# NVIDIA-Genomics-Research/DL4VC

Hardware: AMD Instinct MI355X
Metric: candidate-variants/sec (DAN fwd, 64 reads x 201 bp) (higher is better)
Workload: dtype f32

## Files before the change

dl4vc_amd/config.py:

```python
from __future__ import annotations

from dataclasses import dataclass, field, asdict
from typing import Sequence, Tuple

SINGLE_READ_LENGTH = 201
NUM_SINGLE_READS = 100
MAX_READS = 100
MIN_RESIDUAL_LAYER = 2
MAX_LAYERS = 16
L0_MAX_LAYERS = 12

PRECISION_F32 = 0
PRECISION_BF16X3 = 1
PRECISION_BF16 = 2


class UnsupportedModelOption(ValueError):
    """A Basic2DNet option outside the hot path's scope was requested."""


@dataclass(frozen=True)
class DanConfig:
    reads: int = NUM_SINGLE_READS
    length: int = SINGLE_READ_LENGTH
    layers: int = 7
    c_init: int = 128
    c_final: int = 128
    dil_mid: int = 2
    dil_final: int = 2
    pool_layers: Tuple[int, ...] = (2,)
    residual_start: int = 5
    use_bn: bool = True
    use_q: bool = True
    use_strand: bool = True
    use_mask: bool = True
    bottleneck: int = 32
    fc_sizes: Tuple[int, ...] = (1024, 256)
    embed_dim: int = 20
    precision: int = PRECISION_F32
    conv_algo: int = 0
    skip_empty_rows: bool = False
    bf16_form: int = 0

# ... 24 lines not shown
    @property
    def highway_width(self) -> int:
        return self.layers * self.bottleneck * self.reads

    @property
    def feature_width(self) -> int:
        return self.pooled_width + self.highway_width

    def macs_per_position(self) -> int:
        total = 0
        for l in range(1, self.layers + 1):
            cin, cout, _ = self.layer_dims(l)
            total += 3 * cin * cout
            if self.is_residual(l):
                total += cout * cout
            total += cout * self.bottleneck + self.bottleneck * self.bottleneck
        return total

    def flops_per_site(self) -> float:
        fc = 0
        sizes = (self.feature_width,) + tuple(self.fc_sizes)
        for a, b in zip(sizes[:-1], sizes[1:]):
            fc += a * b
        fc += sizes[-1] * 27
        return 2.0 * (self.reads * self.length * self.macs_per_position() + fc)

    def winograd_applies(self) -> bool:
        dil_ok = (self.layers < 3 or self.dil_mid == 2) and (self.layers < 2 or self.dil_final == 2)
        return self.precision == PRECISION_F32 and dil_ok and self.conv_algo != 1 and self.layers > 1

    def executed_macs_per_position(self) -> float:
        total = float(self.macs_per_position())
        if self.winograd_applies():
            for l in range(2, self.layers + 1):
                cin, cout, _ = self.layer_dims(l)
                total -= cin * cout
        first_segment = min(self.pool_layers) if self.pool_layers else self.layers
        if self.precision == PRECISION_F32 and first_segment <= L0_MAX_LAYERS:
            cin, cout, _ = self.layer_dims(1)
            total -= 3 * cin * cout
        return total

    def input_bytes_per_site(self) -> int:
        return 3 * self.reads * self.length + 3 * self.length

    def to_dict(self):
        return asdict(self)

    def validate(self):
        if not (1 <= self.layers <= MAX_LAYERS):
            raise UnsupportedModelOption("layers must be in 1..%d" % MAX_LAYERS)
        if self.reads < 1 or self.length < 8:
            raise UnsupportedModelOption("reads >= 1 and length >= 8 required")
        if self.residual_start > 0 and self.residual_start < MIN_RESIDUAL_LAYER:
            raise UnsupportedModelOption("Do not allow residuals starting at conv layer %d" % self.residual_start)
        for p in self.pool_layers:
            if not (1 <= p < self.layers):
                raise UnsupportedModelOption("pool layer %d must lie in 1..layers-1" % p)
        if self.layers == 1 and self.c_init != self.c_final:
            raise UnsupportedModelOption("a single conv layer needs init_conv_channels == final_conv_channels")
        if self.bottleneck < 0 or len(self.fc_sizes) != 2:
            raise UnsupportedModelOption("bottleneck >= 0 and exactly two FC layers required")
        if self.conv_algo not in (0, 1, 2):
            raise UnsupportedModelOption("conv_algo must be 0 (auto), 1 (direct) or 2 (winograd)")
        if self.bf16_form not in (0, 1) or (self.bf16_form and self.precision != PRECISION_BF16):
            raise UnsupportedModelOption("bf16_form is 0 or 1 and selects a form of the precision-2 (bf16) kernel")
        if self.embed_dim != 20:
            raise UnsupportedModelOption("embed_dim is fixed at 20 in the reference's scripts")

# ... 39 lines not shown
```

dl4vc_amd/csrc/dan_capi.cpp:

```cpp
#include "../../include/dl4vc_dan.h"
#include "dan_kernels.h"

#include <algorithm>
#include <cmath>
#include <cstdarg>
#include <cstdio>
#include <cstring>
#include <map>
#include <string>
#include <thread>
#include <vector>

using namespace dan;

namespace {

struct Tensor {
    std::vector<float> data;
    std::vector<int64_t> shape;
    int64_t numel() const { int64_t n = 1; for (auto s : shape) n *= s; return n; }
};

std::string g_create_error;

// ... 388 lines not shown
                        v += (double)s.Wf(o, e, t) * emb.data[(size_t)ta * EMBED + e] + (double)s.Wf(o, EMBED + e, t) * emb.data[(size_t)tb * EMBED + e];
                    tab[L0_TJ_OFF + ((size_t)t * L0_NTJ + ta * 10 + tb) * CPAD + o] = (float)v;
                }
            for (int k = 0; k < 5; ++k) tab[L0_WSC_OFF + ((size_t)k * 3 + t) * CPAD + o] = s.Wf(o, 2 * EMBED + k, t);
        }
    std::vector<double> pet((size_t)3 * L * CPAD);
    for (int t = 0; t < 3; ++t)
        for (int wcol = 0; wcol < L; ++wcol)
            for (int o = 0; o < CPAD; ++o) {
                double v = 0.0;
                for (int e = 0; e < EMBED; ++e) v += ((double)s.Wf(o, e, t) + (double)s.Wf(o, EMBED + e, t)) * pe.data[(size_t)wcol * EMBED + e];
                pet[((size_t)t * L + wcol) * CPAD + o] = v;
            }
    for (int var = 0; var < 3; ++var)
        for (int wcol = 0; wcol < L; ++wcol)
            for (int o = 0; o < CPAD; ++o) {
                double v = pet[((size_t)1 * L + wcol) * CPAD + o];
                if (var != 1 && wcol - 1 >= 0) v += pet[((size_t)0 * L + wcol - 1) * CPAD + o];
                if (var != 2 && wcol + 1 < L) v += pet[((size_t)2 * L + wcol + 1) * CPAD + o];
                tab[L0_PE_OFF + ((size_t)var * L + wcol) * CPAD + o] = (float)v;
            }
    return tab;
}

void pack_layer_fp32(const LayerSrc& s, float* blk) {
    auto Wf = [&](int o, int cc, int t) { return s.Wf(o, cc, t); };
    pack_frag(blk + W_OFF, 3, s.l == 0 ? KG0 : KGC, KGC, Wf);
    if (s.l > 0) {
        auto Wu = [&](int o, int cc, int k) -> float {
            const double g0 = s.Wf(o, cc, 0), g1 = s.Wf(o, cc, 1), g2 = s.Wf(o, cc, 2);
            return k == 0 ? (float)g0 : k == 1 ? (float)((g0 + g1 + g2) * 0.5) : k == 2 ? (float)((g0 - g1 + g2) * 0.5) : (float)g2;
        };
        pack_frag(blk + WW_OFF, 4, KGC, KGC, Wu);
    }
    if (s.wr) pack_frag(blk + WRES_OFF, 1, KGC, KGC, [&](int o, int cc, int) { return s.Wr(o, cc); });
    if (s.wb) pack_frag(blk + WBOT_OFF, 1, KGC, 2, [&](int o, int cc, int) { return s.Wb(o, cc); });
}

void pack_layer_bf16p(const LayerSrc& s, const float* cst, char* blkp, char* blkr) {
    auto Wf = [&](int o, int cc, int t) { return s.Wf(o, cc, t); };
    auto Wr = [&](int o, int cc, int) { return s.Wr(o, cc); };
    auto Wb = [&](int o, int cc, int) { return s.Wb(o, cc); };
    pack_fragp((uint16_t*)(blkp + WP_CONV_OFF), 3, s.l == 0 ? P_KS0 : P_KSC, 4, Wf);
    pack_frag16<1>((uint16_t*)(blkr + WP_CONV_OFF), 3, s.l == 0 ? 2 : 4, 8, Wf);
    if (s.wr) {
        pack_fragp((uint16_t*)(blkp + WP_RES_OFF), 1, P_KSC, 4, Wr);
        pack_frag16<1>((uint16_t*)(blkr + WP_RES_OFF), 1, 4, 8, Wr);
    }
    if (s.wb) {
        pack_fragp((uint16_t*)(blkp + WP_BOT_OFF), 1, P_KSC, 1, Wb);
        pack_frag16<1>((uint16_t*)(blkr + WP_BOT_OFF), 1, 4, 2, Wb);
    }
    memcpy(blkp + WP_CST_OFF, cst, CST_FLOATS * sizeof(float));
    memcpy(blkr + WP_CST_OFF, cst, CST_FLOATS * sizeof(float));
}

void pack_layer_bf16x(const LayerSrc& s, const float* cst, char* blkx) {
    pack_frag16<2>((uint16_t*)(blkx + WX_CONV_OFF), 3, s.l == 0 ? X_KS0 : X_KS, 8, [&](int o, int cc, int t) { return s.Wf(o, cc, t); });
    if (s.wr) pack_frag16<2>((uint16_t*)(blkx + WX_RES_OFF), 1, X_KS, 8, [&](int o, int cc, int) { return s.Wr(o, cc); });
    if (s.wb) pack_frag16<2>((uint16_t*)(blkx + WX_BOT_OFF), 1, X_KS, 2, [&](int o, int cc, int) { return s.Wb(o, cc); });
    float* cx = (float*)(blkx + WX_CST_OFF);
    memcpy(cx, cst, CST_FLOATS * sizeof(float));
    for (int ch = 0; ch < CPAD; ++ch) {
        const double b = cx[CST_BIAS + ch];
        cx[CST_SHIFT + ch] = (float)((double)cx[CST_SHIFT + ch] + b * (double)cx[CST_SCALE + ch]);
        cx[CST_BIAS + ch] = (float)-b;
// ... 593 lines not shown
}

int dan_set_tap(dan_t* h, int32_t layer) {
    if (!h) return DAN_ERR_INVALID_ARG;
    if (layer < -1 || layer > h->cfg.layers) return fail(h, DAN_ERR_INVALID_ARG, "tap layer %d out of range", layer);
    if (layer >= 0 && !h->d_tap) {
        if (!h->finalized) return fail(h, DAN_ERR_STATE, "dan_set_tap before dan_finalize");
        HIPCHK(h, hipSetDevice(h->cfg.device_id));
        int rc = dev_alloc(h, &h->d_tap, (size_t)h->chunk * h->cfg.reads * h->cfg.length * CPAD);
        if (rc) return rc;
    }
    h->tap_layer = layer;
    return DAN_OK;
}

int dan_set_pool_form(dan_t* h, int32_t form) {
    if (!h) return DAN_ERR_INVALID_ARG;
    if (form < 0 || form > 2) return fail(h, DAN_ERR_INVALID_ARG, "pool form %d: 0 = automatic, 1 = separate kernels, 2 = in-segment", form);
    if (form == 2 && h->fold_why_not) return fail(h, DAN_ERR_INVALID_ARG, "pool form 2 refused: %s", h->fold_why_not);
    h->pool_form = form;
    h->last_pool_form = (form == 1 || h->fold_why_not) ? 1 : 2;
    return DAN_OK;
}

int64_t dan_query(const dan_t* h, const char* what) {
    if (!h || !what) return DAN_ERR_INVALID_ARG;
    const std::string w(what);
    if (w == "feature_width") return h->F;
    if (w == "feature_stride") return h->F_stride;
    if (w == "chunk_sites") return h->chunk;
    if (w == "chunk_sites_auto") return h->chunk_auto ? 1 : 0;
    if (w == "max_batch") return h->max_batch;
    if (w == "cpad") return CPAD;
    if (w == "tap_sites") return h->last_chunk_sites;
    if (w == "segments") return h->n_segments;
    if (w == "bf16_pingpong") return h->fam == &FAMILIES[2] ? 1 : 0;
    if (w == "bf16x3_split_kernel") return h->fam == &FAMILIES[1] ? 1 : 0;
    if (w == "hidden0_stride") return h->n0_stride;
    if (w == "pool_form") return h->last_pool_form;
    return fail(h, DAN_ERR_INVALID_ARG, "dan_query: unknown key '%s'", what);
}

int64_t dan_read_buffer(dan_t* h, const char* name, float* dst, int64_t capacity) {
    if (!h || !name || !dst || capacity < 0) return DAN_ERR_INVALID_ARG;
    if (!h->finalized) return fail(h, DAN_ERR_STATE, "dan_read_buffer before dan_finalize");
    const dan_config& c = h->cfg;
    const std::string w(name);
    const float* src = nullptr;
    int64_t n = 0;
    if (w == "tap") { if (!h->d_tap) return fail(h, DAN_ERR_STATE, "no tap was requested"); src = h->d_tap; n = (int64_t)h->last_chunk_sites * c.reads * c.length * CPAD; }
    else if (w == "feature") { src = h->d_feat; n = h->last_batch * h->F_stride; }
    else if (w == "hidden0") { src = h->d_hid0; n = h->last_batch * h->n0_stride; }
    else if (w == "hidden1") { src = h->d_hid1; n = h->last_batch * c.fc_sizes[1]; }
    else if (w == "pool") { src = h->d_pool; n = (int64_t)h->last_chunk_sites * c.length * CPAD; }
    else if (w == "h") {
        if (!h->d_h) return fail(h, DAN_ERR_STATE, "the network has no highway bottleneck");
        const int64_t per_layer = (int64_t)h->last_chunk_sites * c.reads * c.length * HPAD;
        const int64_t stride = (int64_t)h->chunk * c.reads * c.length * HPAD;
        if (per_layer == 0) return fail(h, DAN_ERR_STATE, "dan_read_buffer('h') before the first forward");
        if (capacity < per_layer)
            return fail(h, DAN_ERR_INVALID_ARG, "dan_read_buffer('h'): capacity %lld is less than one layer (%lld floats)", (long long)capacity,
                        (long long)per_layer);
        n = std::min<int64_t>(per_layer * c.layers, capacity) / per_layer * per_layer;
        HIPCHK(h, hipSetDevice(c.device_id));
        HIPCHK(h, hipDeviceSynchronize());
        const bool h_bf16 = h->fam->elem_bytes == 2;
        std::vector<uint16_t> tmp(h_bf16 ? (size_t)per_layer : 0);
        for (int64_t l = 0; l * per_layer < n; ++l) {
            if (h_bf16) {
                HIPCHK(h, hipMemcpy(tmp.data(), (const uint16_t*)h->d_h + l * stride, (size_t)per_layer * 2, hipMemcpyDeviceToHost));
                for (int64_t i = 0; i < per_layer; ++i) dst[l * per_layer + i] = bf16_float(tmp[(size_t)i]);
            } else {
                HIPCHK(h, hipMemcpy(dst + l * per_layer, h->d_h + l * stride, (size_t)per_layer * sizeof(float), hipMemcpyDeviceToHost));
            }
        }
        return n;
    }
    else return fail(h, DAN_ERR_INVALID_ARG, "dan_read_buffer: unknown buffer '%s'", name);
    n = std::min(n, capacity);
    HIPCHK(h, hipSetDevice(c.device_id));
    HIPCHK(h, hipDeviceSynchronize());
    HIPCHK(h, hipMemcpy(dst, src, (size_t)n * sizeof(float), hipMemcpyDeviceToHost));
    return n;
}

int dan_profile_enable(dan_t* h, int32_t on) {
// ... 23 lines not shown
```

dl4vc_amd/csrc/dan_device.h:

```cpp
#pragma once
#include "dan_kernels.h"

namespace dan {

typedef float v4f __attribute__((ext_vector_type(4)));

__device__ __forceinline__ v4f mfma16(float a, float b, v4f c) {
    return __builtin_amdgcn_mfma_f32_16x16x4f32(a, b, c, 0, 0, 0);
}

__device__ __forceinline__ v4f splat(float x) { return (v4f){x, x, x, x}; }

typedef const __attribute__((address_space(1))) v4f* gv4f_ptr;

__device__ __forceinline__ float relu1(float v) { return __builtin_amdgcn_fmed3f(v, 0.f, __builtin_inff()); }

__device__ __forceinline__ void gemm_tile(v4f (&acc)[NT], const v4f (&a)[NT], v4f& b, const float* next) {
#pragma unroll
    for (int s = 0; s < 4; ++s)
#pragma unroll
        for (int n = 0; n < NT; ++n) acc[n] = mfma16(a[n][s], b[s], acc[n]);
    b = *(const v4f*)next;
}

__device__ __forceinline__ void conv_gemm(v4f (&acc)[MTW][NT], const float* xs, gv4f_ptr wl, const v4f (&a_first)[NT],
                                          int kg, int ntaps, int dil, int lane, int m_base, int cnt) {
    const int pos = lane & 15, kk = lane >> 4;
    const int total = ntaps * kg;
    const int t0 = (ntaps == 3) ? -dil : 0;
    const float* xrow = xs + (HALO + m_base * 16 + pos) * LDS_S + kk * 4;
    const bool full = cnt == MTW;
    v4f a_nxt[NT], b[MTW];
#pragma unroll
    for (int n = 0; n < NT; ++n) a_nxt[n] = a_first[n];
    {
        const float* xb = xrow + t0 * LDS_S;
#pragma unroll
        for (int m = 0; m < MTW - 1; ++m) b[m] = *(const v4f*)(xb + m * 16 * LDS_S);
        b[MTW - 1] = full ? *(const v4f*)(xb + (MTW - 1) * 16 * LDS_S) : splat(0.f);
    }
    int t = 0, g = 0;
    for (int it = 0; it < total; ++it) {
        v4f a[NT];
#pragma unroll
        for (int n = 0; n < NT; ++n) a[n] = a_nxt[n];
        const int nx = (it + 1 < total) ? it + 1 : it;
#pragma unroll
        for (int n = 0; n < NT; ++n) a_nxt[n] = wl[(size_t)nx * (KGC * 64) + n * 64];
        int tn = t, gn = g + 1;
        if (gn == kg) { gn = 0; ++tn; }
        if (it + 1 == total) { tn = t; gn = g; }
        const float* xn = xrow + (t0 + tn * dil) * LDS_S + gn * 16;
#pragma unroll
        for (int m = 0; m < MTW - 1; ++m) gemm_tile(acc[m], a, b[m], xn + m * 16 * LDS_S);
        __builtin_amdgcn_sched_group_barrier(0x020, NT, 0);
#pragma unroll
        for (int m = 0; m < MTW - 1; ++m) {
            __builtin_amdgcn_sched_group_barrier(0x008, 4 * NT, 0);
            __builtin_amdgcn_sched_group_barrier(0x100, 1, 0);
        }
        if (full) gemm_tile(acc[MTW - 1], a, b[MTW - 1], xn + (MTW - 1) * 16 * LDS_S);
        t = tn; g = gn;
    }
}

template <int NW, bool RANGE = false, int TILES = MT>
__device__ __forceinline__ void bottleneck(const float* xs, const v4f (&wf)[KGC], const float* bbot, float* hrow, int L,
                                           int wave, int lane, int p_lo = 0) {
    constexpr int PSTEP = NW / 2;
    constexpr int NBT = (TILES + PSTEP - 1) / PSTEP;
    lane = (int)__builtin_amdgcn_mbcnt_hi(~0u, __builtin_amdgcn_mbcnt_lo(~0u, 0u));
    asm volatile("" : "+v"(lane));
    const int pos = lane & 15, kk = lane >> 4;
    const int n = wave & 1, p0 = wave >> 1;
    const float* xrow = xs + (HALO + pos) * LDS_S + kk * 4;
    int roff[NBT];
#pragma unroll
    for (int i = 0; i < NBT; ++i) roff[i] = min(p0 + PSTEP * i, TILES - 1) * 16 * LDS_S;
    v4f acc[NBT], b[NBT];
    {
        const v4f bias = *(const v4f*)(bbot + n * 16 + kk * 4);
#pragma unroll
        for (int i = 0; i < NBT; ++i) acc[i] = bias;
    }
#pragma unroll
    for (int i = 0; i < NBT; ++i) b[i] = *(const v4f*)(xrow + roff[i]);
#pragma unroll
    for (int g = 0; g < KGC; ++g) {
        const int gn = (g + 1 < KGC) ? g + 1 : g;
#pragma unroll
        for (int i = 0; i < NBT; ++i) {
#pragma unroll
            for (int s = 0; s < 4; ++s) acc[i] = mfma16(wf[g][s], b[i][s], acc[i]);
            b[i] = *(const v4f*)(xrow + roff[i] + gn * 16);
// ... 14 lines not shown
            *(v4f*)((char*)hrow + (unsigned)(p * HPAD + n * 16 + kk * 4) * 4u) = v;
        }
    }
}

__device__ __forceinline__ void copy_out(const float* xs, float* dst, int lo, int hi, int tid) {
    for (int i = lo * (CPAD / 4) + tid; i < hi * (CPAD / 4); i += SEG_THREADS) {
        const int p = i >> 5, c4 = i & 31;
        ((v4f*)dst)[i] = *(const v4f*)(xs + (HALO + p) * LDS_S + c4 * 4);
    }
}

constexpr int MW = 7;
constexpr int WHB = 102;
constexpr int MW_SHORT = 6;
constexpr int WHB_SHORT = 94;
constexpr int MPOS_SHORT = WHB_SHORT + 16 * MW_SHORT;
constexpr int wino_half_base(int tw) { return tw == MW ? WHB : WHB_SHORT; }
constexpr int wino_cover(int tw) { return tw == MW ? MPOS : MPOS_SHORT; }
template <int TW = MW>
__device__ __forceinline__ int wino_base(int lane) {
    const int n = lane & 15;
    const int c = n & 1, hf = (n >> 2) & 1, q = ((n >> 1) & 1) + 2 * (((n >> 3) ^ (n >> 2)) & 1);
    return hf * wino_half_base(TW) + 4 * q * TW + c;
}

typedef float v2f __attribute__((ext_vector_type(2)));
__device__ __forceinline__ v4f pk_sub(v4f a, v4f b, v2f m1) {
    const v2f lo = __builtin_elementwise_fma((v2f){b[0], b[1]}, m1, (v2f){a[0], a[1]});
    const v2f hi = __builtin_elementwise_fma((v2f){b[2], b[3]}, m1, (v2f){a[2], a[3]});
    return (v4f){lo[0], lo[1], hi[0], hi[1]};
}
__device__ __forceinline__ v4f pk_add(v4f a, v4f b) { return a + b; }
template <int TW, bool REM = false>
__device__ __forceinline__ void conv_gemm_wino(v4f (&acc)[TW][4], const float* xrow, gv4f_ptr wl, const v4f (&a_first)[4],
                                               [[maybe_unused]] v4f& racc, [[maybe_unused]] const float* xr, [[maybe_unused]] gv4f_ptr wd) {
    static_assert(!REM || TW == 6, "the remainder tile's taps follow tiles 1, 3 and 5 of a six-tile walk");
    v4f a_nxt[4];
#pragma unroll
    for (int k = 0; k < 4; ++k) a_nxt[k] = a_first[k];
    v4f xa = *(const v4f*)(xrow), xb = *(const v4f*)(xrow + 2 * LDS_S), xc = *(const v4f*)(xrow + 4 * LDS_S),
        xd = *(const v4f*)(xrow + 6 * LDS_S);
    float neg1 = -1.f;
    asm volatile("" : "+v"(neg1));
    const v2f m1 = {neg1, neg1};
    for (int g = 0; g < KGC; ++g) {
        v4f a[4];
#pragma unroll
        for (int k = 0; k < 4; ++k) a[k] = a_nxt[k];
        const int gn = (g + 1 < KGC) ? g + 1 : g;
#pragma unroll
        for (int k = 0; k < 4; ++k) a_nxt[k] = wl[(size_t)(k * KGC + gn) * (KGC * 64)];
        [[maybe_unused]] v4f ra[3], rb;
        if constexpr (REM) {
#pragma unroll
            for (int t = 0; t < 3; ++t) ra[t] = wd[(size_t)(t * KGC + g) * (KGC * 64)];
        }
        const float* xg = xrow + g * 16;
        const float* xn = xrow + gn * 16;
#pragma unroll
        for (int m = 0; m < TW; ++m) {
            v4f v[4];
            v[0] = pk_sub(xa, xc, m1); v[1] = pk_add(xb, xc); v[2] = pk_sub(xc, xb, m1); v[3] = pk_sub(xb, xd, m1);
            if (m + 1 < TW) {
                xa = xc; xb = xd;
                xc = *(const v4f*)(xg + (4 * m + 8) * LDS_S);
                xd = *(const v4f*)(xg + (4 * m + 10) * LDS_S);
            } else {
                xa = *(const v4f*)(xn); xb = *(const v4f*)(xn + 2 * LDS_S);
                xc = *(const v4f*)(xn + 4 * LDS_S); xd = *(const v4f*)(xn + 6 * LDS_S);
            }
            if constexpr (REM) {
                if ((m & 1) == 0) rb = *(const v4f*)(xr + (m >> 1) * 2 * LDS_S + g * 16);
            }
            __builtin_amdgcn_s_setprio(3);
#pragma unroll
            for (int s = 0; s < 4; ++s)
#pragma unroll
                for (int k = 0; k < 4; ++k) acc[m][k] = mfma16(a[k][s], v[k][s], acc[m][k]);
            if constexpr (REM) {
                if (m & 1) {
#pragma unroll
                    for (int s = 0; s < 4; ++s) racc = mfma16(ra[m >> 1][s], rb[s], racc);
                }
            }
            __builtin_amdgcn_s_setprio(0);
        }
    }
}
template <int TW>
__device__ __forceinline__ void conv_gemm_wino(v4f (&acc)[TW][4], const float* xrow, gv4f_ptr wl, const v4f (&a_first)[4]) {
    v4f none = splat(0.f);
    conv_gemm_wino<TW, false>(acc, xrow, wl, a_first, none, nullptr, nullptr);
}

constexpr int WINO_ROWS_READ = HALO + WHB + 4 * (4 * MW - 1) + 1 + 4 + 1;

}
```

dl4vc_amd/csrc/dan_kernels.h:

```cpp
#pragma once
#include <hip/hip_runtime.h>
#include <stdint.h>

namespace dan {

constexpr int CPAD = 128;
constexpr int NWAVE = 8;
constexpr int SEG_THREADS = NWAVE * 64;
constexpr int NT = 2;
constexpr int MTW = 7;
constexpr int MT = 13;
constexpr int MPOS = MT * 16;
constexpr int HALO = 4;
constexpr int LDS_S = 136;
constexpr int LDS_ROWS = MPOS + 2 * HALO;
constexpr int HPAD = 32;
constexpr int CIN0 = 48;
constexpr int KG0 = CIN0 / 16;
constexpr int KGC = CPAD / 16;
constexpr int EMBED = 20;
constexpr int VOCAB = 10;
constexpr int NHEAD = 27;

constexpr int W_OFF = 0;
constexpr int WRES_OFF = W_OFF + 3 * KGC * KGC * 256;
constexpr int WBOT_OFF = WRES_OFF + KGC * KGC * 256;
constexpr int CST_OFF = WBOT_OFF + KGC * 2 * 256;
constexpr int CST_BIAS = 0, CST_SCALE = CPAD, CST_SHIFT = 2 * CPAD, CST_BRES = 3 * CPAD, CST_BBOT = 4 * CPAD;
constexpr int CST_FLOATS = 4 * CPAD + HPAD;
constexpr int WW_OFF = CST_OFF + CST_FLOATS + 32;
constexpr int LAYER_STRIDE = WW_OFF + 4 * KGC * KGC * 256;
constexpr int MAX_LAYERS = 16;

struct SegmentArgs {
    const float* wl;
    int l_begin, l_end;
    int n_layers;
    int dil_mid, dil_final;
    unsigned res_mask;
    int has_hw;
    int R, L;
    const uint8_t *reads, *qual, *strand, *ref, *ref_mask, *var_mask;
    const float* emb;
    const float* pe;
    float* y;
    const float* pool;
    float* h;
    long long h_layer_stride;
    float* tap;
    int tap_layer;
    int wino;
    int n_rows;
    int xcd_rows;
    const int* work;
    const int* work_count;
    const float* l0_tab;
    int units, Lw;
    int u_off[2], u_len[2], own_lo[2], own_hi[2];
    float* y_out;
    int fold;
    int n_sites, xcd_sites;
    float* fold_scratch;
    float* fold_pool;
    float* fold_feat;
// ... 142 lines not shown
```

dl4vc_amd/csrc/dan_kernels.hip:

```cpp
#include "dan_device.h"
#include "dan_reduce.h"

namespace dan {

#ifdef DAN_STAMPS
__device__ unsigned long long* g_stamps;
constexpr int NSTAMP = 64;
#define STAMP(k)                                                                                      \
    do {                                                                                              \
        __builtin_amdgcn_sched_barrier(0);                                                            \
        unsigned long long t_ = __builtin_amdgcn_s_memtime();                                         \
        __builtin_amdgcn_s_waitcnt(0xC07F);                                                           \
        if (lane == 0 && (k) < NSTAMP) g_stamps[((size_t)stamp_row * NWAVE + wave) * NSTAMP + (k)] = t_; \
        __builtin_amdgcn_sched_barrier(0);                                                            \
    } while (0)
#else
#define STAMP(k) do {} while (0)
#endif

static_assert((HALO + WHB + 4 * (4 * MW - 1) + 1 + 4 + 1) * LDS_S <= LDS_ROWS * LDS_S + MAX_LAYERS * CST_FLOATS, "wino reads stay inside LDS");
static_assert(WHB + 4 * (4 * MW - 1) + 3 >= MPOS - 1 && 4 * (4 * MW - 1) + 3 >= WHB - 1, "wino tiling covers the read");
static_assert(HALO + MPOS_SHORT + 15 + 2 < LDS_ROWS && MPOS_SHORT + 16 <= MPOS, "the remainder tile's taps stay inside the image");
static_assert(WHB_SHORT + 4 * (4 * MW_SHORT - 1) + 3 >= MPOS_SHORT - 1 && 4 * (4 * MW_SHORT - 1) + 3 >= WHB_SHORT - 1 && WHB_SHORT % 4 == 2,
              "short wino tiling covers its unit");
// ... 11 lines not shown
    for (int g = 0; g < KGC; ++g) {
        const v4f a = a_nxt;
        const int gn = (g + 1 < KGC) ? g + 1 : g;
        a_nxt = wl[(size_t)gn * (KGC * 64)];
#pragma unroll
        for (int m = 0; m < TW; ++m) {
            __builtin_amdgcn_s_setprio(3);
#pragma unroll
            for (int s = 0; s < 4; ++s)
#pragma unroll
                for (int o = 0; o < 2; ++o) acc[m][o] = mfma16(a[s], b[m][o][s], acc[m][o]);
            if constexpr (REM) {
                if (m + 1 == TW) {
#pragma unroll
                    for (int s = 0; s < 4; ++s) racc = mfma16(a[s], rb[s], racc);
                }
            }
            __builtin_amdgcn_s_setprio(0);
#pragma unroll
            for (int o = 0; o < 2; ++o) b[m][o] = *(const v4f*)(xrow + (4 * m + 2 * o) * LDS_S + gn * 16);
            if constexpr (REM) {
                if (m + 1 == TW) rb = *(const v4f*)(xr + gn * 16);
            }
        }
    }
}

template <bool WINO, bool PERSIST, bool SPLIT, int TW = MW, bool FOLD = false, bool REM = false>
__global__ __launch_bounds__(SEG_THREADS, NWAVE / 4) void segment_kernel(SegmentArgs a_by_value) {
    static_assert(!FOLD || (PERSIST && !SPLIT), "the site-owning form is a persistent one-unit form");
    static_assert(TW == MW ? !(SPLIT && WINO) : (WINO && TW == MW_SHORT), "six tiles per lane: Winograd forms only, and the split one always");
    static_assert(!REM || (WINO && !SPLIT && TW == MW_SHORT), "the remainder tile [190, 206): beside six Winograd tiles of a one-unit read");
    constexpr int TILES = (SPLIT && WINO) ? (MPOS_SHORT + 15) / 16 : MT;
    __shared__ __attribute__((aligned(16))) float lds[LDS_ROWS * LDS_S + MAX_LAYERS * CST_FLOATS];
    float* const xs = lds;
    float* const cst = lds + LDS_ROWS * LDS_S;
    typedef const __attribute__((address_space(4))) SegmentArgs* kernarg_ptr;
    constexpr int UNITS = SPLIT ? 2 : 1;
    const int n_work = FOLD ? a_by_value.n_sites : (a_by_value.work_count ? *a_by_value.work_count : a_by_value.n_rows) * UNITS;
    const int per = FOLD ? a_by_value.xcd_sites : a_by_value.work_count ? (n_work + 7) >> 3 : a_by_value.xcd_rows * UNITS;
    const int xcd = blockIdx.x & 7;
    int j = blockIdx.x >> 3;
    int wk = xcd * per + j;
    if (j >= per || wk >= n_work) return;
    [[maybe_unused]] int fold_r = 0;
next_row:
    {
    kernarg_ptr ap = (kernarg_ptr)__builtin_amdgcn_kernarg_segment_ptr();
    if (PERSIST) asm volatile("" : "+s"(ap));
    auto args = [&]() -> decltype(auto) { if constexpr (PERSIST) return (*ap); else return (a_by_value); };
    const auto& a = args();
    [[maybe_unused]] const int unit = wk & 1;
    const int L = SPLIT ? (unit ? a.u_len[1] : a.u_len[0]) : a.L;
    const int Lw = SPLIT ? a.Lw : L;
    const int u_off = SPLIT ? (unit ? a.u_off[1] : a.u_off[0]) : 0;
    [[maybe_unused]] const int own_lo = SPLIT ? (unit ? a.own_lo[1] : a.own_lo[0]) : 0;
    [[maybe_unused]] const int own_hi = SPLIT ? (unit ? a.own_hi[1] : a.own_hi[0]) : L;
    [[maybe_unused]] const int stamp_row = wk;
    int tid = threadIdx.x;
    if (PERSIST) asm volatile("" : "+v"(tid));
    const int lane = tid & 63;
    const int wave = __builtin_amdgcn_readfirstlane(tid >> 6);
    const int wrow = SPLIT ? wk >> 1 : wk;
    const int row_index = FOLD ? wk * a.R + fold_r : __builtin_amdgcn_readfirstlane(a.work_count ? a.work[wrow] : wrow);
    const int site = FOLD ? wk : (int)((unsigned)row_index / (unsigned)a.R);
    const int r = FOLD ? fold_r : row_index - site * a.R;
    const size_t read_idx = (size_t)site * a.R + r;
    float* yrow = a.y + (read_idx * (size_t)Lw + u_off) * CPAD;
    float* yout = SPLIT ? a.y_out + (read_idx * (size_t)Lw + u_off) * CPAD : yrow;
    const int pos = lane & 15, kk = lane >> 4;
    const int cq = wave & 3, ph = wave >> 2;
    const int m_base = ph * MTW, cnt = ph ? MT - MTW : MTW;
    int chb[NT];
#pragma unroll
    for (int n = 0; n < NT; ++n) chb[n] = (cq * NT + n) * 16 + kk * 4;

    STAMP(0);
    [[maybe_unused]] const int wP0 = wino_base<TW>(lane);
    [[maybe_unused]] const int wlim = ((lane >> 2) & 1) ? wino_cover(TW) : wino_half_base(TW);
    [[maybe_unused]] const int chw = wave * 16 + kk * 4;
    auto dil_of = [&](int l) { return (l == 0) ? 1 : (l + 1 < a.n_layers ? a.dil_mid : a.dil_final); };
    auto wino_layer = [&](int l) { return WINO && l > 0; };
    constexpr bool CARRY = !(WINO && PERSIST);
    v4f pc0 = splat(0.f), pc1 = pc0, pc2 = pc0, pc3 = pc0, pn0 = pc0, pn1 = pc0, pn2 = pc0, pn3 = pc0;
    auto first_frags = [&](int l, v4f& f0, v4f& f1, v4f& f2, v4f& f3) {
        const float* blk = a.wl + (size_t)l * LAYER_STRIDE;
        if (wino_layer(l)) {
            gv4f_ptr w0 = (gv4f_ptr)(blk + WW_OFF) + wave * 64 + lane;
            constexpr size_t KS = (size_t)KGC * (KGC * 64);
            f0 = w0[0]; f1 = w0[KS]; f2 = w0[2 * KS]; f3 = w0[3 * KS];
        } else {
            gv4f_ptr w0 = (gv4f_ptr)(blk + W_OFF) + (cq * NT) * 64 + lane;
            f0 = w0[0]; f1 = w0[64];
        }
    };
    const bool l0_lookup = a.l_begin == 0 && a.l0_tab != nullptr && !(a.tap && a.tap_layer == 0) && (a.l_end - a.l_begin) <= L0_MAX_LAYERS;
    float* const tokf = cst + (a.l_end - a.l_begin) * CST_FLOATS;
    if ((!WINO || a.l_begin == 0) && !l0_lookup) first_frags(a.l_begin, pc0, pc1, pc2, pc3);
    auto stage_constants = [&]() {
        for (int i = tid; i < (a.l_end - a.l_begin) * CST_FLOATS; i += SEG_THREADS) {
            const int l = i / CST_FLOATS, j = i - l * CST_FLOATS;
            cst[i] = a.wl[(size_t)(a.l_begin + l) * LAYER_STRIDE + CST_OFF + j];
        }
    };

    if (a.l_begin == 0) {
        if (l0_lookup) {
            for (int i = tid; i < (LDS_ROWS - L) * (LDS_S / 4); i += SEG_THREADS) {
                const int rr = i / (LDS_S / 4), c4 = i - rr * (LDS_S / 4);
                const int row = rr < HALO ? rr : rr + L;
                *(v4f*)(xs + row * LDS_S + c4 * 4) = splat(0.f);
            }
        } else {
            for (int i = tid; i < LDS_ROWS * LDS_S / 4; i += SEG_THREADS) ((v4f*)xs)[i] = splat(0.f);
        }
        stage_constants();
// ... 100 lines not shown
        STAMP(sb + 7);
        if (CARRY) { pc0 = pn0; pc1 = pn1; pc2 = pn2; pc3 = pn3; }
    };

    auto direct_layer = [&](int l) {
        const float* wblk = a.wl + (size_t)l * LAYER_STRIDE;
        const float* lc = cst + (l - a.l_begin) * CST_FLOATS;
        const bool residual = (a.res_mask >> l) & 1u;
        const int kg = (l == 0) ? KG0 : KGC;
        const int dil = dil_of(l);
        gv4f_ptr w_conv = (gv4f_ptr)(wblk + W_OFF) + (cq * NT) * 64 + lane;
        gv4f_ptr w_res = (gv4f_ptr)(wblk + WRES_OFF) + (cq * NT) * 64 + lane;
        gv4f_ptr w_bot = (gv4f_ptr)(wblk + WBOT_OFF) + lane;
        [[maybe_unused]] const int sb = 2 + (l - a.l_begin) * 8;
        if (!WINO && l + 1 < a.l_end) first_frags(l + 1, pn0, pn1, pn2, pn3);
        const bool from_global = (l == a.l_begin) && (a.l_begin != 0) && (a.pool != nullptr);
        v4f pre_res[NT];
#pragma unroll
        for (int n = 0; n < NT; ++n) pre_res[n] = residual ? w_res[n * 64] : splat(0.f);
        static_assert(NT == 2, "two direct-form fragments are carried");
        const v4f pre_dir[NT] = {pc0, pc1};

        v4f acc[MTW][NT];
        {
            v4f bias[NT];
#pragma unroll
            for (int n = 0; n < NT; ++n) bias[n] = *(const v4f*)(lc + CST_BIAS + chb[n]);
#pragma unroll
            for (int m = 0; m < MTW; ++m)
#pragma unroll
                for (int n = 0; n < NT; ++n) acc[m][n] = bias[n];
        }
        STAMP(sb + 0);
        conv_gemm(acc, xs, w_conv, pre_dir, kg, 3, dil, lane, m_base, cnt);
        STAMP(sb + 1);
        const bool bot_here = a.has_hw && !(WINO && l + 1 < a.l_end);
        if (bot_here && !residual) {
#pragma unroll
            for (int g = 0; g < KGC; ++g) wbot[g] = w_bot[(g * 2 + (wave & 1)) * 64];
        }
        {
            v4f sc[NT], sh[NT];
#pragma unroll
            for (int n = 0; n < NT; ++n) { sc[n] = *(const v4f*)(lc + CST_SCALE + chb[n]); sh[n] = *(const v4f*)(lc + CST_SHIFT + chb[n]); }
#pragma unroll
            for (int m = 0; m < MTW; ++m) {
                const bool live = ((m_base + m) * 16 + pos) < L;
#pragma unroll
                for (int n = 0; n < NT; ++n) {
                    v4f v = acc[m][n];
#pragma unroll
                    for (int j = 0; j < 4; ++j) v[j] = live ? relu1(v[j]) * sc[n][j] + sh[n][j] : 0.f;
                    acc[m][n] = v;
                }
            }
        }
        STAMP(sb + 2);
        __syncthreads();
        STAMP(sb + 3);
        if (residual) {
            v4f bres[NT];
#pragma unroll
            for (int n = 0; n < NT; ++n) bres[n] = *(const v4f*)(lc + CST_BRES + chb[n]);
            if (!from_global) {
#pragma unroll
                for (int m = 0; m < MTW; ++m) {
                    if (m < cnt) {
// ... 37 lines not shown
                    for (int n = 0; n < NT; ++n) *(v4f*)(xs + (HALO + p) * LDS_S + chb[n]) = (p < L) ? acc[m][n] : splat(0.f);
                }
            }
        } else {
#pragma unroll
            for (int m = 0; m < MTW; ++m) {
                if (m < cnt) {
#pragma unroll
                    for (int n = 0; n < NT; ++n)
                        *(v4f*)(xs + (HALO + (m_base + m) * 16 + pos) * LDS_S + chb[n]) = acc[m][n];
                }
            }
        }
        layer_tail(l, lc, true);
    };

    [[maybe_unused]] auto wino_layer_body = [&](int l) {
        if constexpr (WINO) {
        const float* wblk = a.wl + (size_t)l * LAYER_STRIDE;
        const float* lc = cst + (l - a.l_begin) * CST_FLOATS;
        const bool residual = (a.res_mask >> l) & 1u;
        gv4f_ptr w_bot = (gv4f_ptr)(wblk + WBOT_OFF) + lane;
        [[maybe_unused]] const int sb = 2 + (l - a.l_begin) * 8;
        const bool from_global = (l == a.l_begin) && (a.l_begin != 0) && (a.pool != nullptr);
        gv4f_ptr w_w = (gv4f_ptr)(wblk + WW_OFF) + wave * 64 + lane;
        gv4f_ptr w_r1 = (gv4f_ptr)(wblk + WRES_OFF) + wave * 64 + lane;
        float* xw = xs + (HALO + wP0) * LDS_S;
        v4f out[TW][2], pre_r1;
        [[maybe_unused]] v4f rout = splat(0.f);
        [[maybe_unused]] int rp = MPOS_SHORT + pos;
        int wp = wP0;
        float* xq;
        {
            v4f acc[TW][4];
            const v4f bias = *(const v4f*)(lc + CST_BIAS + chw);
#pragma unroll
            for (int m = 0; m < TW; ++m) { acc[m][0] = splat(0.f); acc[m][1] = bias; acc[m][2] = splat(0.f); acc[m][3] = splat(0.f); }
            if constexpr (REM) rout = bias;
            STAMP(sb + 0);
            auto gemm = [&](const v4f (&pre_w)[4]) {
                if constexpr (REM)
                    conv_gemm_wino<TW, true>(acc, xw - 2 * LDS_S + kk * 4, w_w, pre_w, rout, xs + (HALO + rp - 2) * LDS_S + kk * 4, (gv4f_ptr)(wblk + W_OFF) + wave * 64 + lane);
                else
                    conv_gemm_wino(acc, xw - 2 * LDS_S + kk * 4, w_w, pre_w);
            };
            if constexpr (CARRY) {
                const v4f pre_w[4] = {pc0, pc1, pc2, pc3};
                gemm(pre_w);
            } else {
                gv4f_ptr w0 = w_w;
                const v4f pre_w[4] = {w0[0], w0[(size_t)KGC * (KGC * 64)], w0[(size_t)2 * KGC * (KGC * 64)], w0[(size_t)3 * KGC * (KGC * 64)]};
                gemm(pre_w);
            }
            STAMP(sb + 1);
            asm volatile("" : "+v"(wp));
            if constexpr (REM) asm volatile("" : "+v"(rp));
            xq = xs + (HALO + wp) * LDS_S;
            const v4f sc = *(const v4f*)(lc + CST_SCALE + chw), sh = *(const v4f*)(lc + CST_SHIFT + chw);
            const v2f sc_lo = {sc[0], sc[1]}, sc_hi = {sc[2], sc[3]}, sh_lo = {sh[0], sh[1]}, sh_hi = {sh[2], sh[3]};
            auto half = [](v4f v, int h) { return (v2f){v[2 * h], v[2 * h + 1]}; };
            v2f neg1 = {-1.f, -1.f};
            asm volatile("" : "+v"(neg1));
            auto act = [](v2f y, v2f s, v2f t) {
                const v2f r = {relu1(y[0]), relu1(y[1])};
                return __builtin_elementwise_fma(r, s, t);
            };
#pragma unroll
            for (int m = 0; m < TW; ++m) {
                const v2f y0l = half(acc[m][0], 0) + half(acc[m][1], 0) + half(acc[m][2], 0), y0h = half(acc[m][0], 1) + half(acc[m][1], 1) + half(acc[m][2], 1);
                const v2f y1l = __builtin_elementwise_fma(half(acc[m][3], 0), neg1, __builtin_elementwise_fma(half(acc[m][2], 0), neg1, half(acc[m][1], 0)));
                const v2f y1h = __builtin_elementwise_fma(half(acc[m][3], 1), neg1, __builtin_elementwise_fma(half(acc[m][2], 1), neg1, half(acc[m][1], 1)));
                const v2f o0l = act(y0l, sc_lo, sh_lo), o0h = act(y0h, sc_hi, sh_hi), o1l = act(y1l, sc_lo, sh_lo), o1h = act(y1h, sc_hi, sh_hi);
                out[m][0] = (v4f){o0l[0], o0l[1], o0h[0], o0h[1]};
                out[m][1] = (v4f){o1l[0], o1l[1], o1h[0], o1h[1]};
            }
            if constexpr (REM) {
                const v2f rl = act(half(rout, 0), sc_lo, sh_lo), rh = act(half(rout, 1), sc_hi, sh_hi);
                rout = (v4f){rl[0], rl[1], rh[0], rh[1]};
            }
        }
        [[maybe_unused]] float* const rcell = xs + (HALO + rp) * LDS_S + chw;
        int wl = min(wlim, L);
        asm volatile("" : "+v"(wl));
        __builtin_amdgcn_sched_barrier(0);
        pre_r1 = residual ? w_r1[0] : splat(0.f);
        if (CARRY && !residual && l + 1 < a.l_end) first_frags(l + 1, pn0, pn1, pn2, pn3);
        if (a.has_hw && l > a.l_begin && wave < NWAVE / 2) {
            gv4f_ptr w_bp = (gv4f_ptr)(wblk - LAYER_STRIDE + WBOT_OFF) + lane;
#pragma unroll
            for (int g = 0; g < KGC; ++g) wbot[g] = w_bp[(g * 2 + (wave & 1)) * 64];
            bottleneck<NWAVE / 2, SPLIT, TILES>(xs, wbot, lc - CST_FLOATS + CST_BBOT,
                                         a.h + (size_t)(l - 1) * a.h_layer_stride + (read_idx * (size_t)Lw + u_off) * HPAD, own_hi, wave, lane, own_lo);
        }
        const bool bot_here = a.has_hw && !(l + 1 < a.l_end);
        if (bot_here && !residual) {
#pragma unroll
            for (int g = 0; g < KGC; ++g) wbot[g] = w_bot[(g * 2 + (wave & 1)) * 64];
        }
        STAMP(sb + 2);
        __syncthreads();
        STAMP(sb + 3);
        if (residual) {
            const v4f bres = *(const v4f*)(lc + CST_BRES + chw);
            if (from_global) {
#pragma unroll
                for (int m = 0; m < TW; ++m)
#pragma unroll
// ... 639 lines not shown
```

Measured before the change: 14310.

## Use Winograd F(4,3) for short-read dilated conv layers in place of F(2,3)

```diff
diff --git a/dl4vc_amd/config.py b/dl4vc_amd/config.py
--- a/dl4vc_amd/config.py
+++ b/dl4vc_amd/config.py
@@ -9,6 +9,7 @@
 MIN_RESIDUAL_LAYER = 2
 MAX_LAYERS = 16
 L0_MAX_LAYERS = 12
+WINO_F43_MAX_LENGTH = 206
 
 PRECISION_F32 = 0
 PRECISION_BF16X3 = 1
@@ -99,9 +100,10 @@
     def executed_macs_per_position(self) -> float:
         total = float(self.macs_per_position())
         if self.winograd_applies():
+            saved = 1.5 if self.length <= WINO_F43_MAX_LENGTH else 1.0
             for l in range(2, self.layers + 1):
                 cin, cout, _ = self.layer_dims(l)
-                total -= cin * cout
+                total -= saved * cin * cout
         first_segment = min(self.pool_layers) if self.pool_layers else self.layers
         if self.precision == PRECISION_F32 and first_segment <= L0_MAX_LAYERS:
             cin, cout, _ = self.layer_dims(1)
diff --git a/dl4vc_amd/csrc/dan_capi.cpp b/dl4vc_amd/csrc/dan_capi.cpp
--- a/dl4vc_amd/csrc/dan_capi.cpp
+++ b/dl4vc_amd/csrc/dan_capi.cpp
@@ -444,6 +444,18 @@
             return k == 0 ? (float)g0 : k == 1 ? (float)((g0 + g1 + g2) * 0.5) : k == 2 ? (float)((g0 - g1 + g2) * 0.5) : (float)g2;
         };
         pack_frag(blk + WW_OFF, 4, KGC, KGC, Wu);
+        auto Wu43 = [&](int o, int cc, int k) -> float {
+            const double g0 = s.Wf(o, cc, 0), g1 = s.Wf(o, cc, 1), g2 = s.Wf(o, cc, 2);
+            switch (k) {
+                case 0: return (float)(g0 / 4.0);
+                case 1: return (float)(-(g0 + g1 + g2) / 6.0);
+                case 2: return (float)(-(g0 - g1 + g2) / 6.0);
+                case 3: return (float)(g0 / 24.0 + g1 / 12.0 + g2 / 6.0);
+                case 4: return (float)(g0 / 24.0 - g1 / 12.0 + g2 / 6.0);
+                default: return (float)g2;
+            }
+        };
+        pack_frag(blk + W43_OFF, 6, KGC, KGC, Wu43);
     }
     if (s.wr) pack_frag(blk + WRES_OFF, 1, KGC, KGC, [&](int o, int cc, int) { return s.Wr(o, cc); });
     if (s.wb) pack_frag(blk + WBOT_OFF, 1, KGC, 2, [&](int o, int cc, int) { return s.Wb(o, cc); });
@@ -1103,6 +1115,9 @@
     if (w == "chunk_sites_auto") return h->chunk_auto ? 1 : 0;
     if (w == "max_batch") return h->max_batch;
     if (w == "cpad") return CPAD;
+    if (w == "layer_stride") return LAYER_STRIDE;
+    if (w == "wino_f23_offset") return WW_OFF;
+    if (w == "wino_f43_offset") return W43_OFF;
     if (w == "tap_sites") return h->last_chunk_sites;
     if (w == "segments") return h->n_segments;
     if (w == "bf16_pingpong") return h->fam == &FAMILIES[2] ? 1 : 0;
@@ -1123,6 +1138,10 @@
     else if (w == "feature") { src = h->d_feat; n = h->last_batch * h->F_stride; }
     else if (w == "hidden0") { src = h->d_hid0; n = h->last_batch * h->n0_stride; }
     else if (w == "hidden1") { src = h->d_hid1; n = h->last_batch * c.fc_sizes[1]; }
+    else if (w == "wl") {
+        if (!h->d_wl) return fail(h, DAN_ERR_STATE, "dan_read_buffer('wl'): this precision keeps no fp32 weight blocks");
+        src = h->d_wl; n = (int64_t)c.layers * LAYER_STRIDE;
+    }
     else if (w == "pool") { src = h->d_pool; n = (int64_t)h->last_chunk_sites * c.length * CPAD; }
     else if (w == "h") {
         if (!h->d_h) return fail(h, DAN_ERR_STATE, "the network has no highway bottleneck");
diff --git a/dl4vc_amd/csrc/dan_device.h b/dl4vc_amd/csrc/dan_device.h
--- a/dl4vc_amd/csrc/dan_device.h
+++ b/dl4vc_amd/csrc/dan_device.h
@@ -23,6 +23,7 @@
     b = *(const v4f*)next;
 }
 
+template <bool JOIN_WAIT = false>
 __device__ __forceinline__ void conv_gemm(v4f (&acc)[MTW][NT], const float* xs, gv4f_ptr wl, const v4f (&a_first)[NT],
                                           int kg, int ntaps, int dil, int lane, int m_base, int cnt) {
     const int pos = lane & 15, kk = lane >> 4;
@@ -60,6 +61,10 @@
             __builtin_amdgcn_sched_group_barrier(0x100, 1, 0);
         }
         if (full) gemm_tile(acc[MTW - 1], a, b[MTW - 1], xn + (MTW - 1) * 16 * LDS_S);
+        if constexpr (JOIN_WAIT) {
+            asm volatile("s_nop 7");
+            __builtin_amdgcn_sched_barrier(0);
+        }
         t = tn; g = gn;
     }
 }
@@ -140,10 +145,8 @@
     return (v4f){lo[0], lo[1], hi[0], hi[1]};
 }
 __device__ __forceinline__ v4f pk_add(v4f a, v4f b) { return a + b; }
-template <int TW, bool REM = false>
-__device__ __forceinline__ void conv_gemm_wino(v4f (&acc)[TW][4], const float* xrow, gv4f_ptr wl, const v4f (&a_first)[4],
-                                               [[maybe_unused]] v4f& racc, [[maybe_unused]] const float* xr, [[maybe_unused]] gv4f_ptr wd) {
-    static_assert(!REM || TW == 6, "the remainder tile's taps follow tiles 1, 3 and 5 of a six-tile walk");
+template <int TW>
+__device__ __forceinline__ void conv_gemm_wino(v4f (&acc)[TW][4], const float* xrow, gv4f_ptr wl, const v4f (&a_first)[4]) {
     v4f a_nxt[4];
 #pragma unroll
     for (int k = 0; k < 4; ++k) a_nxt[k] = a_first[k];
@@ -159,11 +162,6 @@
         const int gn = (g + 1 < KGC) ? g + 1 : g;
 #pragma unroll
         for (int k = 0; k < 4; ++k) a_nxt[k] = wl[(size_t)(k * KGC + gn) * (KGC * 64)];
-        [[maybe_unused]] v4f ra[3], rb;
-        if constexpr (REM) {
-#pragma unroll
-            for (int t = 0; t < 3; ++t) ra[t] = wd[(size_t)(t * KGC + g) * (KGC * 64)];
-        }
         const float* xg = xrow + g * 16;
         const float* xn = xrow + gn * 16;
 #pragma unroll
@@ -178,28 +176,81 @@
                 xa = *(const v4f*)(xn); xb = *(const v4f*)(xn + 2 * LDS_S);
                 xc = *(const v4f*)(xn + 4 * LDS_S); xd = *(const v4f*)(xn + 6 * LDS_S);
             }
+            __builtin_amdgcn_s_setprio(3);
+#pragma unroll
+            for (int s = 0; s < 4; ++s)
+#pragma unroll
+                for (int k = 0; k < 4; ++k) acc[m][k] = mfma16(a[k][s], v[k][s], acc[m][k]);
+            __builtin_amdgcn_s_setprio(0);
+        }
+    }
+}
+
+constexpr int MW43 = MW_SHORT / 2;
+__device__ __forceinline__ v4f pk_fma(v4f a, v2f k, v4f c) {
+    const v2f lo = __builtin_elementwise_fma((v2f){a[0], a[1]}, k, (v2f){c[0], c[1]});
+    const v2f hi = __builtin_elementwise_fma((v2f){a[2], a[3]}, k, (v2f){c[2], c[3]});
+    return (v4f){lo[0], lo[1], hi[0], hi[1]};
+}
+template <bool REM>
+__device__ __forceinline__ void conv_gemm_wino43(v4f (&acc)[MW43][6], const float* xrow, gv4f_ptr wl, const v4f (&a_first)[6],
+                                                 [[maybe_unused]] v4f& racc, [[maybe_unused]] const float* xr, [[maybe_unused]] gv4f_ptr wd) {
+    v4f a_nxt[6], d[6];
+#pragma unroll
+    for (int k = 0; k < 6; ++k) a_nxt[k] = a_first[k];
+#pragma unroll
+    for (int i = 0; i < 6; ++i) d[i] = *(const v4f*)(xrow + 2 * i * LDS_S);
+    [[maybe_unused]] v4f rb;
+    if constexpr (REM) rb = *(const v4f*)xr;
+    float c1 = -1.f, c2 = 2.f, c4 = 4.f, c5 = -5.f;
+    asm volatile("" : "+v"(c1), "+v"(c2), "+v"(c4), "+v"(c5));
+    const v2f m1 = {c1, c1}, p2 = {c2, c2}, m2 = {-c2, -c2}, p4 = {c4, c4}, m4 = {-c4, -c4}, m5 = {c5, c5};
+    for (int g = 0; g < KGC; ++g) {
+        v4f a[6];
+#pragma unroll
+        for (int k = 0; k < 6; ++k) a[k] = a_nxt[k];
+        const int gn = (g + 1 < KGC) ? g + 1 : g;
+#pragma unroll
+        for (int k = 0; k < 6; ++k) a_nxt[k] = wl[(size_t)(k * KGC + gn) * (KGC * 64)];
+        [[maybe_unused]] v4f ra[3];
+        if constexpr (REM) {
+#pragma unroll
+            for (int t = 0; t < 3; ++t) ra[t] = wd[(size_t)(t * KGC + g) * (KGC * 64)];
+        }
+        const float* xg = xrow + g * 16;
+        const float* xn = xrow + gn * 16;
+#pragma unroll
+        for (int m = 0; m < MW43; ++m) {
+            v4f v[6];
+            {
+                const v4f a42 = pk_fma(d[2], m4, d[4]), b31 = pk_fma(d[1], m4, d[3]);
+                const v4f c42 = pk_fma(d[2], m1, d[4]), e31 = pk_fma(d[1], m1, d[3]);
+                v[0] = pk_fma(d[2], m5, pk_fma(d[0], p4, d[4]));
+                v[1] = pk_add(a42, b31); v[2] = pk_fma(b31, m1, a42);
+                v[3] = pk_fma(e31, p2, c42); v[4] = pk_fma(e31, m2, c42);
+                v[5] = pk_fma(d[3], m5, pk_fma(d[1], p4, d[5]));
+            }
+            if (m + 1 < MW43) {
+                d[0] = d[4]; d[1] = d[5];
+#pragma unroll
+                for (int i = 2; i < 6; ++i) d[i] = *(const v4f*)(xg + (8 * (m + 1) + 2 * i) * LDS_S);
+            } else {
+#pragma unroll
+                for (int i = 0; i < 6; ++i) d[i] = *(const v4f*)(xn + 2 * i * LDS_S);
+            }
+            __builtin_amdgcn_s_setprio(3);
+#pragma unroll
+            for (int s = 0; s < 4; ++s)
+#pragma unroll
+                for (int k = 0; k < 6; ++k) acc[m][k] = mfma16(a[k][s], v[k][s], acc[m][k]);
             if constexpr (REM) {
-                if ((m & 1) == 0) rb = *(const v4f*)(xr + (m >> 1) * 2 * LDS_S + g * 16);
-            }
-            __builtin_amdgcn_s_setprio(3);
-#pragma unroll
-            for (int s = 0; s < 4; ++s)
-#pragma unroll
-                for (int k = 0; k < 4; ++k) acc[m][k] = mfma16(a[k][s], v[k][s], acc[m][k]);
-            if constexpr (REM) {
-                if (m & 1) {
-#pragma unroll
-                    for (int s = 0; s < 4; ++s) racc = mfma16(ra[m >> 1][s], rb[s], racc);
-                }
+#pragma unroll
+                for (int s = 0; s < 4; ++s) racc = mfma16(ra[m][s], rb[s], racc);
             }
             __builtin_amdgcn_s_setprio(0);
-        }
-    }
-}
-template <int TW>
-__device__ __forceinline__ void conv_gemm_wino(v4f (&acc)[TW][4], const float* xrow, gv4f_ptr wl, const v4f (&a_first)[4]) {
-    v4f none = splat(0.f);
-    conv_gemm_wino<TW, false>(acc, xrow, wl, a_first, none, nullptr, nullptr);
+            if constexpr (REM) rb = *(const v4f*)(m + 1 < MW43 ? xr + (m + 1) * 2 * LDS_S + g * 16 : xr + gn * 16);
+        }
+    }
 }
 
 constexpr int WINO_ROWS_READ = HALO + WHB + 4 * (4 * MW - 1) + 1 + 4 + 1;
diff --git a/dl4vc_amd/csrc/dan_kernels.h b/dl4vc_amd/csrc/dan_kernels.h
--- a/dl4vc_amd/csrc/dan_kernels.h
+++ b/dl4vc_amd/csrc/dan_kernels.h
@@ -29,7 +29,8 @@
 constexpr int CST_BIAS = 0, CST_SCALE = CPAD, CST_SHIFT = 2 * CPAD, CST_BRES = 3 * CPAD, CST_BBOT = 4 * CPAD;
 constexpr int CST_FLOATS = 4 * CPAD + HPAD;
 constexpr int WW_OFF = CST_OFF + CST_FLOATS + 32;
-constexpr int LAYER_STRIDE = WW_OFF + 4 * KGC * KGC * 256;
+constexpr int W43_OFF = WW_OFF + 4 * KGC * KGC * 256;
+constexpr int LAYER_STRIDE = W43_OFF + 6 * KGC * KGC * 256;
 constexpr int MAX_LAYERS = 16;
 
 struct SegmentArgs {
diff --git a/dl4vc_amd/csrc/dan_kernels.hip b/dl4vc_amd/csrc/dan_kernels.hip
--- a/dl4vc_amd/csrc/dan_kernels.hip
+++ b/dl4vc_amd/csrc/dan_kernels.hip
@@ -67,6 +67,7 @@
     static_assert(TW == MW ? !(SPLIT && WINO) : (WINO && TW == MW_SHORT), "six tiles per lane: Winograd forms only, and the split one always");
     static_assert(!REM || (WINO && !SPLIT && TW == MW_SHORT), "the remainder tile [190, 206): beside six Winograd tiles of a one-unit read");
     constexpr int TILES = (SPLIT && WINO) ? (MPOS_SHORT + 15) / 16 : MT;
+    constexpr bool W43 = WINO && !SPLIT && TW == MW_SHORT;
     __shared__ __attribute__((aligned(16))) float lds[LDS_ROWS * LDS_S + MAX_LAYERS * CST_FLOATS];
     float* const xs = lds;
     float* const cst = lds + LDS_ROWS * LDS_S;
@@ -116,7 +117,7 @@
     [[maybe_unused]] const int chw = wave * 16 + kk * 4;
     auto dil_of = [&](int l) { return (l == 0) ? 1 : (l + 1 < a.n_layers ? a.dil_mid : a.dil_final); };
     auto wino_layer = [&](int l) { return WINO && l > 0; };
-    constexpr bool CARRY = !(WINO && PERSIST);
+    constexpr bool CARRY = !(WINO && (PERSIST || W43));
     v4f pc0 = splat(0.f), pc1 = pc0, pc2 = pc0, pc3 = pc0, pn0 = pc0, pn1 = pc0, pn2 = pc0, pn3 = pc0;
     auto first_frags = [&](int l, v4f& f0, v4f& f1, v4f& f2, v4f& f3) {
         const float* blk = a.wl + (size_t)l * LAYER_STRIDE;
@@ -283,7 +284,7 @@
                 for (int n = 0; n < NT; ++n) acc[m][n] = bias[n];
         }
         STAMP(sb + 0);
-        conv_gemm(acc, xs, w_conv, pre_dir, kg, 3, dil, lane, m_base, cnt);
+        conv_gemm<W43>(acc, xs, w_conv, pre_dir, kg, 3, dil, lane, m_base, cnt);
         STAMP(sb + 1);
         const bool bot_here = a.has_hw && !(WINO && l + 1 < a.l_end);
         if (bot_here && !residual) {
@@ -387,25 +388,27 @@
         int wp = wP0;
         float* xq;
         {
-            v4f acc[TW][4];
+            constexpr int NTL = W43 ? MW43 : TW, NCP = W43 ? 6 : 4;
+            v4f acc[NTL][NCP];
             const v4f bias = *(const v4f*)(lc + CST_BIAS + chw);
 #pragma unroll
-            for (int m = 0; m < TW; ++m) { acc[m][0] = splat(0.f); acc[m][1] = bias; acc[m][2] = splat(0.f); acc[m][3] = splat(0.f); }
+            for (int m = 0; m < NTL; ++m)
+#pragma unroll
+                for (int k = 0; k < NCP; ++k) acc[m][k] = (k == 1) ? bias : splat(0.f);
             if constexpr (REM) rout = bias;
             STAMP(sb + 0);
-            auto gemm = [&](const v4f (&pre_w)[4]) {
-                if constexpr (REM)
-                    conv_gemm_wino<TW, true>(acc, xw - 2 * LDS_S + kk * 4, w_w, pre_w, rout, xs + (HALO + rp - 2) * LDS_S + kk * 4, (gv4f_ptr)(wblk + W_OFF) + wave * 64 + lane);
-                else
-                    conv_gemm_wino(acc, xw - 2 * LDS_S + kk * 4, w_w, pre_w);
-            };
-            if constexpr (CARRY) {
+            if constexpr (W43) {
+                gv4f_ptr w0 = (gv4f_ptr)(wblk + W43_OFF) + wave * 64 + lane;
+                constexpr size_t KS = (size_t)KGC * (KGC * 64);
+                const v4f pre_w[6] = {w0[0], w0[KS], w0[2 * KS], w0[3 * KS], w0[4 * KS], w0[5 * KS]};
+                conv_gemm_wino43<REM>(acc, xw - 2 * LDS_S + kk * 4, w0, pre_w, rout, xs + (HALO + rp - 2) * LDS_S + kk * 4, (gv4f_ptr)(wblk + W_OFF) + wave * 64 + lane);
+            } else if constexpr (CARRY) {
                 const v4f pre_w[4] = {pc0, pc1, pc2, pc3};
-                gemm(pre_w);
+                conv_gemm_wino(acc, xw - 2 * LDS_S + kk * 4, w_w, pre_w);
             } else {
                 gv4f_ptr w0 = w_w;
                 const v4f pre_w[4] = {w0[0], w0[(size_t)KGC * (KGC * 64)], w0[(size_t)2 * KGC * (KGC * 64)], w0[(size_t)3 * KGC * (KGC * 64)]};
-                gemm(pre_w);
+                conv_gemm_wino(acc, xw - 2 * LDS_S + kk * 4, w_w, pre_w);
             }
             STAMP(sb + 1);
             asm volatile("" : "+v"(wp));
@@ -420,14 +423,38 @@
                 const v2f r = {relu1(y[0]), relu1(y[1])};
                 return __builtin_elementwise_fma(r, s, t);
             };
-#pragma unroll
-            for (int m = 0; m < TW; ++m) {
-                const v2f y0l = half(acc[m][0], 0) + half(acc[m][1], 0) + half(acc[m][2], 0), y0h = half(acc[m][0], 1) + half(acc[m][1], 1) + half(acc[m][2], 1);
-                const v2f y1l = __builtin_elementwise_fma(half(acc[m][3], 0), neg1, __builtin_elementwise_fma(half(acc[m][2], 0), neg1, half(acc[m][1], 0)));
-                const v2f y1h = __builtin_elementwise_fma(half(acc[m][3], 1), neg1, __builtin_elementwise_fma(half(acc[m][2], 1), neg1, half(acc[m][1], 1)));
-                const v2f o0l = act(y0l, sc_lo, sh_lo), o0h = act(y0h, sc_hi, sh_hi), o1l = act(y1l, sc_lo, sh_lo), o1h = act(y1h, sc_hi, sh_hi);
-                out[m][0] = (v4f){o0l[0], o0l[1], o0h[0], o0h[1]};
-                out[m][1] = (v4f){o1l[0], o1l[1], o1h[0], o1h[1]};
+            if constexpr (W43) {
+                v2f c2 = {2.f, 2.f}, c4 = {4.f, 4.f}, c8 = {8.f, 8.f};
+                asm volatile("" : "+v"(c2), "+v"(c4), "+v"(c8));
+#pragma unroll
+                for (int m = 0; m < MW43; ++m) {
+                    v2f y[4][2];
+#pragma unroll
+                    for (int h = 0; h < 2; ++h) {
+                        const v2f M0 = half(acc[m][0], h), M1 = half(acc[m][1], h), M2 = half(acc[m][2], h), M3 = half(acc[m][3], h), M4 = half(acc[m][4], h),
+                                  M5 = half(acc[m][5], h);
+                        const v2f s1 = M1 + M2, d1 = __builtin_elementwise_fma(M2, neg1, M1), s2 = M3 + M4, d2 = __builtin_elementwise_fma(M4, neg1, M3);
+                        y[0][h] = M0 + s1 + s2;
+                        y[1][h] = __builtin_elementwise_fma(d2, c2, d1);
+                        y[2][h] = __builtin_elementwise_fma(s2, c4, s1);
+                        y[3][h] = __builtin_elementwise_fma(d2, c8, d1) + M5;
+                    }
+#pragma unroll
+                    for (int o = 0; o < 4; ++o) {
+                        const v2f lo = act(y[o][0], sc_lo, sh_lo), hi = act(y[o][1], sc_hi, sh_hi);
+                        out[2 * m + (o >> 1)][o & 1] = (v4f){lo[0], lo[1], hi[0], hi[1]};
+                    }
+                }
+            } else {
+#pragma unroll
+                for (int m = 0; m < TW; ++m) {
+                    const v2f y0l = half(acc[m][0], 0) + half(acc[m][1], 0) + half(acc[m][2], 0), y0h = half(acc[m][0], 1) + half(acc[m][1], 1) + half(acc[m][2], 1);
+                    const v2f y1l = __builtin_elementwise_fma(half(acc[m][3], 0), neg1, __builtin_elementwise_fma(half(acc[m][2], 0), neg1, half(acc[m][1], 0)));
+                    const v2f y1h = __builtin_elementwise_fma(half(acc[m][3], 1), neg1, __builtin_elementwise_fma(half(acc[m][2], 1), neg1, half(acc[m][1], 1)));
+                    const v2f o0l = act(y0l, sc_lo, sh_lo), o0h = act(y0h, sc_hi, sh_hi), o1l = act(y1l, sc_lo, sh_lo), o1h = act(y1h, sc_hi, sh_hi);
+                    out[m][0] = (v4f){o0l[0], o0l[1], o0h[0], o0h[1]};
+                    out[m][1] = (v4f){o1l[0], o1l[1], o1h[0], o1h[1]};
+                }
             }
             if constexpr (REM) {
                 const v2f rl = act(half(rout, 0), sc_lo, sh_lo), rh = act(half(rout, 1), sc_hi, sh_hi);
```

Result: faster. 15230, median of 6 (+6.5%).
